# MaxHalford/sorobn

Measured on NVIDIA H100. Metric: exact-inference queries/sec, higher is better.
Workload: dtype f32

## Files before the change

### sorobn_b200/csrc/sbn_join.cu

```cuda
#include "sbn_join.h"

#include <cuda.h>

#include <algorithm>
#include <cstring>

#include "sbn_internal.h"
#include "sbn_kernels.cuh"
#include "sbn_launch.h"
#include "sbn_tma.h"

namespace {

constexpr int kT = 5;
constexpr int kSmemMax = 220 * 1024;

struct SbnJoinParams {
    CUtensorMap tm[SBN_JOIN_MAX_BATCHED];
    SbnStep s;
    int32_t boff[SBN_MAX_IN];
    int32_t map_in[SBN_JOIN_MAX_BATCHED];
    int32_t n_maps;
    int32_t rows;
    int32_t stage_floats;
    uint32_t stage_bytes;
    int32_t n_blocks;
};

__device__ __forceinline__ void tma_3d(float *dst, const CUtensorMap *map, int32_t row, uint64_t *bar) {
    asm volatile("cp.async.bulk.tensor.3d.shared::cluster.global.mbarrier::complete_tx::bytes [%0], [%1, {%3, %4, %4}], [%2];" ::"r"(
                     sbn_smem_u32(dst)),
                 "l"(reinterpret_cast<uint64_t>(map)), "r"(sbn_smem_u32(bar)), "r"(row), "r"(0)
                 : "memory");
}

template <int NU, int NA, int NB>
__global__ void __launch_bounds__(SBN_JOIN_MAX_THREADS, 1) sbn_join_kernel(const __grid_constant__ SbnJoinParams p) {
    constexpr int T = kT, CX = kT, S = SBN_JOIN_STAGES;
    constexpr int N_IN = NU + NA + NB;
    constexpr int TB = NB > 0 ? T : 1;
    constexpr int ROW_WORDS = N_IN + 2;
    const SbnStep &s = p.s;
    extern __shared__ __align__(128) float s_mem[];
    __shared__ __align__(8) uint64_t s_full[S], s_tab;
    sbn_pdl_launch_dependents();

    const int R = p.rows;
    float *const tab = s_mem + S * p.stage_floats;
    const bool staged = s.smem_floats > 0;
    if (threadIdx.x == 0) {
#pragma unroll
        for (int k = 0; k < S; ++k) sbn_mbar_init(&s_full[k], 1);
        sbn_mbar_init(&s_tab, 1);
        sbn_fence_mbar_init();
    }
    __syncthreads();
    if (threadIdx.x == 0 && staged) {
        sbn_mbar_expect_tx(&s_tab, static_cast<uint32_t>(s.smem_floats) * 4u);
#pragma unroll
        for (int i = 0; i < N_IN; ++i)
            if (!s.in[i].batched) sbn_tma_bulk_g2s(tab + s.in[i].smem_off, s.in[i].ptr, static_cast<uint32_t>(s.in[i].stage_floats) * 4u, &s_tab);
    }
    auto issue = [&](int stage, int blk) {
        float *const dst = s_mem + stage * p.stage_floats;
        sbn_mbar_expect_tx(&s_full[stage], p.stage_bytes);
        for (int m = 0; m < p.n_maps; ++m) tma_3d(dst + p.boff[p.map_in[m]], &p.tm[m], blk * R, &s_full[stage]);
    };
    sbn_pdl_wait();
    if (threadIdx.x == 0)
        for (int k = 0; k < S; ++k)
            if (blockIdx.x + k * gridDim.x < p.n_blocks) issue(k, blockIdx.x + k * gridDim.x);

    const int r = threadIdx.x % R, t = threadIdx.x / R;
    const int32_t *const row = s.tile_off + static_cast<int64_t>(t) * ROW_WORDS;
    const int o_base = __ldg(row);
    int base[N_IN];
#pragma unroll
    for (int i = 0; i < N_IN; ++i) base[i] = __ldg(row + 2 + i);
    const int c0 = s.card[0];
    const int cx = s.cx;
    if (staged) sbn_mbar_wait(&s_tab, 0);

    for (int it = 0, blk = blockIdx.x; blk < p.n_blocks; ++it, blk += gridDim.x) {
        const int stage = it % S;
        const int b = blk * R + r;
        const bool live = b < s.n_rows;
        const float *src[N_IN];
        int mul[N_IN];
        const float *const stg = s_mem + stage * p.stage_floats;
#pragma unroll
        for (int i = 0; i < N_IN; ++i) {
            if (s.in[i].batched) {
                src[i] = stg + p.boff[i] + r;
                mul[i] = R;
            } else {
                int e = s.in[i].smem_off;
                for (int k = 0; k < s.in[i].n_ev; ++k) {
                    const int code = live ? min(static_cast<int>(s.ev[static_cast<int64_t>(s.in[i].ev_col[k]) * s.ld_ev + b]), s.in[i].ev_card[k] - 1) : 0;
                    e += code * s.in[i].ev_stride[k];
                }
                src[i] = tab + e;
                mul[i] = 1;
            }
        }
        sbn_mbar_wait(&s_full[stage], static_cast<uint32_t>((it / S) & 1));

        float acc[T][TB];
#pragma unroll
        for (int d0 = 0; d0 < T; ++d0)
#pragma unroll
            for (int d1 = 0; d1 < TB; ++d1) acc[d0][d1] = 0.f;
        for (int xo = 0; xo < cx; xo += CX) {
            int ob[N_IN];
#pragma unroll
            for (int i = 0; i < N_IN; ++i) ob[i] = base[i] + __ldg(s.zoff + i * cx + xo);
#pragma unroll
            for (int x = 0; x < CX; ++x) {
                float a[T], bb[TB];
#pragma unroll
                for (int d = 0; d < T; ++d) {
                    float v = 1.f;
#pragma unroll
                    for (int j = 0; j < NA; ++j) {
                        const int i = NU + j;
                        const float r_ = src[i][(ob[i] + x * s.in[i].sx + d * s.in[i].stride[0]) * mul[i]];
                        v = (j == 0) ? r_ : v * r_;
                    }
#pragma unroll
                    for (int i = 0; i < NU; ++i) v *= src[i][(ob[i] + x * s.in[i].sx) * mul[i]];
                    a[d] = v;
                }
#pragma unroll
                for (int d = 0; d < TB; ++d) {
                    float v = 1.f;
#pragma unroll
                    for (int j = 0; j < NB; ++j) {
                        const int i = NU + NA + j;
                        const float r_ = src[i][(ob[i] + x * s.in[i].sx + d * s.in[i].stride[1]) * mul[i]];
                        v = (j == 0) ? r_ : v * r_;
                    }
                    bb[d] = v;
                }
#pragma unroll
                for (int d0 = 0; d0 < T; ++d0)
#pragma unroll
                    for (int d1 = 0; d1 < TB; ++d1) acc[d0][d1] = fmaf(a[d0], bb[d1], acc[d0][d1]);
            }
        }
        if (live) {
#pragma unroll
            for (int d1 = 0; d1 < TB; ++d1)
#pragma unroll
                for (int d0 = 0; d0 < T; ++d0) __stcs(s.out + static_cast<int64_t>(o_base + d1 * c0 + d0) * s.ld + b, acc[d0][d1]);
        }
        __syncthreads();
        if (threadIdx.x == 0 && blk + S * static_cast<int>(gridDim.x) < p.n_blocks) issue(stage, blk + S * gridDim.x);
    }
}

#define SBN_JOIN_COMBOS(X) \
    X(0, 1, 0) X(0, 1, 1) X(0, 1, 2) X(0, 2, 0) X(0, 2, 1) X(1, 1, 0) X(1, 1, 1) X(1, 2, 0) X(2, 1, 0) X(2, 1, 1)

bool instantiated(int nu, int na, int nb) {
#define SBN_JOIN_HAS(U, A, B) \
    if (nu == U && na == A && nb == B) return true;
    SBN_JOIN_COMBOS(SBN_JOIN_HAS)
#undef SBN_JOIN_HAS
    return false;
}

struct JoinShape {
    int rows = 0;
    int stage_floats = 0;
    uint32_t stage_bytes = 0;
    size_t smem = 0;
    int32_t boff[SBN_MAX_IN] = {};
    int e_lo[SBN_MAX_IN] = {};
};

int split_entries(int64_t n) {
    for (int d = 256; d >= 1; --d)
        if (n % d == 0) return n / d <= 256 ? d : 0;
    return 0;
}

bool shape_of(const sbn_program *P, const StepDesc &st, const SbnStep &q, JoinShape *js) {
    if (P->f64 || !P->use_tiled || !P->use_preload) return false;
    if (st.kind != 1 || st.tile != kT || st.nc != 0 || q.tile_off == nullptr || q.zoff == nullptr || q.cx_inner != kT || q.cx % kT != 0)
        return false;
    if (q.slab_off != nullptr || q.slices != nullptr || q.norm_out != nullptr) return false;
    if (!(st.in.size() <= 3 || (st.nu == 2 && st.na == 1 && st.nb == 1)) || !instantiated(st.nu, st.na, st.nb)) return false;
    const int64_t n_tiles = st.n_tiles;
    const int tb = st.nb > 0 ? kT : 1;
    for (int64_t t = 0; t < n_tiles; ++t)
        if (P->h_tile_words[static_cast<size_t>(st.tile_off_pos + t * (q.n_in + 2) + 1)] != (kT | tb << 8)) return false;
    const int rows = n_tiles * 16 >= 128 ? 16 : 32;
    if (n_tiles * rows < 128 || n_tiles * rows > SBN_JOIN_MAX_THREADS) return false;
    int n_batched = 0;
    int64_t stage = 0;
    for (int i = 0; i < q.n_in; ++i) {
        const InDesc &in = st.in[st.order[i]];
        if (!in.batched) {
            if (q.in[i].smem_off < 0) return false;
            continue;
        }
        if (++n_batched > SBN_JOIN_MAX_BATCHED) return false;
        const int64_t n_e = P->slots[in.id].size;
        js->e_lo[i] = split_entries(n_e);
        if (js->e_lo[i] == 0) return false;
        js->boff[i] = static_cast<int32_t>(stage);
        stage += round_up(n_e * rows, 32);
        js->stage_bytes += static_cast<uint32_t>(n_e * rows * 4);
    }
    if (n_batched != SBN_JOIN_MAX_BATCHED) return false;
    js->rows = rows;
    js->stage_floats = static_cast<int>(stage);
    js->smem = static_cast<size_t>(SBN_JOIN_STAGES * stage + q.smem_floats) * 4;
    if (js->smem > kSmemMax) return false;
    return q.n_rows >= 2LL * P->n_sms * rows;
}

template <int NU, int NA, int NB>
cudaError_t set_attr() {
    return cudaFuncSetAttribute(sbn_join_kernel<NU, NA, NB>, cudaFuncAttributeMaxDynamicSharedMemorySize, kSmemMax);
}

}

int sbn_join_rows(const sbn_program *P, const StepDesc &st, const SbnStep &q) {
    JoinShape js;
    return shape_of(P, st, q, &js) ? js.rows : 0;
}

cudaError_t sbn_join_set_attrs() {
    cudaError_t e = cudaSuccess;
#define SBN_JOIN_ATTR(U, A, B) \
    if (e == cudaSuccess) e = set_attr<U, A, B>();
    SBN_JOIN_COMBOS(SBN_JOIN_ATTR)
#undef SBN_JOIN_ATTR
    return e;
}

cudaError_t sbn_join_launch(sbn_program *P, const StepDesc &st, const SbnStep &q, cudaStream_t stream) {
    JoinShape js;
    if (!shape_of(P, st, q, &js)) return cudaErrorInvalidValue;
    SbnJoinParams p;
    memset(&p, 0, sizeof p);
    p.s = q;
    p.rows = js.rows;
    p.stage_floats = js.stage_floats;
    p.stage_bytes = js.stage_bytes;
    p.n_blocks = static_cast<int32_t>((q.n_rows + js.rows - 1) / js.rows);
    for (int i = 0; i < q.n_in; ++i) {
        p.boff[i] = js.boff[i];
        if (!q.in[i].batched) continue;
        const int64_t n_e = P->slots[st.in[st.order[i]].id].size;
        if (!sbn_tma_encode_rows(&p.tm[p.n_maps], q.in[i].ptr, q.ld, q.n_rows, n_e, js.rows, js.e_lo[i])) return cudaErrorInvalidValue;
        p.map_in[p.n_maps++] = i;
    }
    const dim3 g(static_cast<unsigned>(std::min<int64_t>(p.n_blocks, P->n_sms))), b(static_cast<unsigned>(js.rows * st.n_tiles));
    const int key = st.nu * 100 + st.na * 10 + st.nb;
    switch (key) {
#define SBN_JOIN_CASE(U, A, B)                                                \
    case U * 100 + A * 10 + B:                                                \
        sbn_launch(sbn_join_kernel<U, A, B>, g, b, js.smem, stream, p);       \
        break;
        SBN_JOIN_COMBOS(SBN_JOIN_CASE)
#undef SBN_JOIN_CASE
        default: return cudaErrorInvalidValue;
    }
    return cudaGetLastError();
}
```

Measured before the change: 26.53 million.

## Stage join outputs in shared memory and write them with TMA bulk stores

Output tiles are now written into a shared-memory box and sent to global memory with a TMA tensor store, replacing per-thread streaming stores. The next block's inputs are prefetched into L2 with TMA, and evidence columns are prefetched with prefetch.global.L2. Addressing is also rewritten to precomputed byte offsets with strength-reduced x increments. This uses more shared memory, adds an extra __syncthreads per block, and requires the output entry count to be splittable.

Result: faster. 27.33 million, median of 6 (+3.0%).

```diff
diff --git a/sorobn_b200/csrc/sbn_join.cu b/sorobn_b200/csrc/sbn_join.cu
--- a/sorobn_b200/csrc/sbn_join.cu
+++ b/sorobn_b200/csrc/sbn_join.cu
@@ -17,12 +17,14 @@
 
 struct SbnJoinParams {
     CUtensorMap tm[SBN_JOIN_MAX_BATCHED];
+    CUtensorMap tm_out;
     SbnStep s;
     int32_t boff[SBN_MAX_IN];
     int32_t map_in[SBN_JOIN_MAX_BATCHED];
     int32_t n_maps;
     int32_t rows;
     int32_t stage_floats;
+    int32_t out_floats;
     uint32_t stage_bytes;
     int32_t n_blocks;
 };
@@ -32,6 +34,18 @@
                      sbn_smem_u32(dst)),
                  "l"(reinterpret_cast<uint64_t>(map)), "r"(sbn_smem_u32(bar)), "r"(row), "r"(0)
                  : "memory");
+}
+
+__device__ __forceinline__ void tma_prefetch_3d(const CUtensorMap *map, int32_t row) {
+    asm volatile("cp.async.bulk.prefetch.tensor.3d.L2.global [%0, {%1, %2, %2}];" ::"l"(reinterpret_cast<uint64_t>(map)), "r"(row), "r"(0)
+                 : "memory");
+}
+
+__device__ __forceinline__ void tma_store_3d(const CUtensorMap *map, const float *src, int32_t row) {
+    asm volatile("cp.async.bulk.tensor.3d.global.shared::cta.bulk_group [%0, {%2, %3, %3}], [%1];" ::"l"(reinterpret_cast<uint64_t>(map)),
+                 "r"(sbn_smem_u32(src)), "r"(row), "r"(0)
+                 : "memory");
+    asm volatile("cp.async.bulk.commit_group;" ::: "memory");
 }
 
 template <int NU, int NA, int NB>
@@ -46,7 +60,8 @@
     sbn_pdl_launch_dependents();
 
     const int R = p.rows;
-    float *const tab = s_mem + S * p.stage_floats;
+    float *const obox = s_mem + S * p.stage_floats;
+    float *const tab = obox + p.out_floats;
     const bool staged = s.smem_floats > 0;
     if (threadIdx.x == 0) {
 #pragma unroll
@@ -66,41 +81,60 @@
         sbn_mbar_expect_tx(&s_full[stage], p.stage_bytes);
         for (int m = 0; m < p.n_maps; ++m) tma_3d(dst + p.boff[p.map_in[m]], &p.tm[m], blk * R, &s_full[stage]);
     };
+    auto prefetch = [&](int blk) {
+        for (int m = 0; m < p.n_maps; ++m) tma_prefetch_3d(&p.tm[m], blk * R);
+    };
     sbn_pdl_wait();
-    if (threadIdx.x == 0)
+    if (threadIdx.x == 0) {
         for (int k = 0; k < S; ++k)
             if (blockIdx.x + k * gridDim.x < p.n_blocks) issue(k, blockIdx.x + k * gridDim.x);
+        if (blockIdx.x + S * gridDim.x < p.n_blocks) prefetch(blockIdx.x + S * gridDim.x);
+    }
 
     const int r = threadIdx.x % R, t = threadIdx.x / R;
     const int32_t *const row = s.tile_off + static_cast<int64_t>(t) * ROW_WORDS;
     const int o_base = __ldg(row);
-    int base[N_IN];
-#pragma unroll
-    for (int i = 0; i < N_IN; ++i) base[i] = __ldg(row + 2 + i);
+    const int tab_b = static_cast<int>(tab - s_mem) * 4;
+    int tile_b[N_IN], mb[N_IN], xs_b[N_IN], ds_b[N_IN];
+    const int32_t *zp[N_IN];
+#pragma unroll
+    for (int i = 0; i < N_IN; ++i) {
+        const bool bat = s.in[i].batched != 0;
+        mb[i] = bat ? 4 * R : 4;
+        tile_b[i] = __ldg(row + 2 + i) * mb[i] + (bat ? (p.boff[i] + r) * 4 : tab_b + s.in[i].smem_off * 4);
+        xs_b[i] = s.in[i].sx * mb[i];
+        ds_b[i] = (i < NU ? 0 : i < NU + NA ? s.in[i].stride[0] : s.in[i].stride[1]) * mb[i];
+        zp[i] = s.zoff + i * s.cx;
+    }
     const int c0 = s.card[0];
     const int cx = s.cx;
+    const char *const smc = reinterpret_cast<const char *>(s_mem);
+    auto ld = [&](int off) { return *reinterpret_cast<const float *>(smc + off); };
     if (staged) sbn_mbar_wait(&s_tab, 0);
 
     for (int it = 0, blk = blockIdx.x; blk < p.n_blocks; ++it, blk += gridDim.x) {
         const int stage = it % S;
         const int b = blk * R + r;
         const bool live = b < s.n_rows;
-        const float *src[N_IN];
-        int mul[N_IN];
-        const float *const stg = s_mem + stage * p.stage_floats;
+        if (t == 0 && b + static_cast<int>(gridDim.x) * R < s.n_rows) {
+#pragma unroll
+            for (int i = 0; i < N_IN; ++i)
+                if (!s.in[i].batched)
+                    for (int k = 0; k < s.in[i].n_ev; ++k)
+                        asm volatile("prefetch.global.L2 [%0];" ::"l"(s.ev + static_cast<int64_t>(s.in[i].ev_col[k]) * s.ld_ev + b + gridDim.x * R));
+        }
+        int blk_off[N_IN];
 #pragma unroll
         for (int i = 0; i < N_IN; ++i) {
             if (s.in[i].batched) {
-                src[i] = stg + p.boff[i] + r;
-                mul[i] = R;
+                blk_off[i] = tile_b[i] + stage * p.stage_floats * 4;
             } else {
-                int e = s.in[i].smem_off;
+                int e = 0;
                 for (int k = 0; k < s.in[i].n_ev; ++k) {
                     const int code = live ? min(static_cast<int>(s.ev[static_cast<int64_t>(s.in[i].ev_col[k]) * s.ld_ev + b]), s.in[i].ev_card[k] - 1) : 0;
                     e += code * s.in[i].ev_stride[k];
                 }
-                src[i] = tab + e;
-                mul[i] = 1;
+                blk_off[i] = tile_b[i] + e * 4;
             }
         }
         sbn_mbar_wait(&s_full[stage], static_cast<uint32_t>((it / S) & 1));
@@ -113,7 +147,7 @@
         for (int xo = 0; xo < cx; xo += CX) {
             int ob[N_IN];
 #pragma unroll
-            for (int i = 0; i < N_IN; ++i) ob[i] = base[i] + __ldg(s.zoff + i * cx + xo);
+            for (int i = 0; i < N_IN; ++i) ob[i] = blk_off[i] + __ldg(zp[i] + xo) * mb[i];
 #pragma unroll
             for (int x = 0; x < CX; ++x) {
                 float a[T], bb[TB];
@@ -123,11 +157,11 @@
 #pragma unroll
                     for (int j = 0; j < NA; ++j) {
                         const int i = NU + j;
-                        const float r_ = src[i][(ob[i] + x * s.in[i].sx + d * s.in[i].stride[0]) * mul[i]];
+                        const float r_ = ld(ob[i] + d * ds_b[i]);
                         v = (j == 0) ? r_ : v * r_;
                     }
 #pragma unroll
-                    for (int i = 0; i < NU; ++i) v *= src[i][(ob[i] + x * s.in[i].sx) * mul[i]];
+                    for (int i = 0; i < NU; ++i) v *= ld(ob[i]);
                     a[d] = v;
                 }
 #pragma unroll
@@ -136,7 +170,7 @@
 #pragma unroll
                     for (int j = 0; j < NB; ++j) {
                         const int i = NU + NA + j;
-                        const float r_ = src[i][(ob[i] + x * s.in[i].sx + d * s.in[i].stride[1]) * mul[i]];
+                        const float r_ = ld(ob[i] + d * ds_b[i]);
                         v = (j == 0) ? r_ : v * r_;
                     }
                     bb[d] = v;
@@ -145,17 +179,26 @@
                 for (int d0 = 0; d0 < T; ++d0)
 #pragma unroll
                     for (int d1 = 0; d1 < TB; ++d1) acc[d0][d1] = fmaf(a[d0], bb[d1], acc[d0][d1]);
+#pragma unroll
+                for (int i = 0; i < N_IN; ++i) ob[i] += xs_b[i];
             }
         }
-        if (live) {
-#pragma unroll
-            for (int d1 = 0; d1 < TB; ++d1)
-#pragma unroll
-                for (int d0 = 0; d0 < T; ++d0) __stcs(s.out + static_cast<int64_t>(o_base + d1 * c0 + d0) * s.ld + b, acc[d0][d1]);
-        }
+        if (threadIdx.x == 0) asm volatile("cp.async.bulk.wait_group.read 0;" ::: "memory");
         __syncthreads();
-        if (threadIdx.x == 0 && blk + S * static_cast<int>(gridDim.x) < p.n_blocks) issue(stage, blk + S * gridDim.x);
-    }
+        if (threadIdx.x == 0) {
+            const int nxt = blk + S * static_cast<int>(gridDim.x);
+            if (nxt < p.n_blocks) issue(stage, nxt);
+            if (nxt + static_cast<int>(gridDim.x) < p.n_blocks) prefetch(nxt + gridDim.x);
+        }
+#pragma unroll
+        for (int d1 = 0; d1 < TB; ++d1)
+#pragma unroll
+            for (int d0 = 0; d0 < T; ++d0) obox[(o_base + d1 * c0 + d0) * R + r] = acc[d0][d1];
+        asm volatile("fence.proxy.async.shared::cta;" ::: "memory");
+        __syncthreads();
+        if (threadIdx.x == 0) tma_store_3d(&p.tm_out, obox, blk * R);
+    }
+    if (threadIdx.x == 0) asm volatile("cp.async.bulk.wait_group 0;" ::: "memory");
 }
 
 #define SBN_JOIN_COMBOS(X) \
@@ -176,6 +219,8 @@
     size_t smem = 0;
     int32_t boff[SBN_MAX_IN] = {};
     int e_lo[SBN_MAX_IN] = {};
+    int out_lo = 0;
+    int out_floats = 0;
 };
 
 int split_entries(int64_t n) {
@@ -215,7 +260,10 @@
     if (n_batched != SBN_JOIN_MAX_BATCHED) return false;
     js->rows = rows;
     js->stage_floats = static_cast<int>(stage);
-    js->smem = static_cast<size_t>(SBN_JOIN_STAGES * stage + q.smem_floats) * 4;
+    js->out_lo = split_entries(q.n_out);
+    if (js->out_lo == 0) return false;
+    js->out_floats = static_cast<int>(round_up(static_cast<int64_t>(q.n_out) * rows, 32));
+    js->smem = static_cast<size_t>(SBN_JOIN_STAGES * stage + js->out_floats + q.smem_floats) * 4;
     if (js->smem > kSmemMax) return false;
     return q.n_rows >= 2LL * P->n_sms * rows;
 }
@@ -258,6 +306,8 @@
         if (!sbn_tma_encode_rows(&p.tm[p.n_maps], q.in[i].ptr, q.ld, q.n_rows, n_e, js.rows, js.e_lo[i])) return cudaErrorInvalidValue;
         p.map_in[p.n_maps++] = i;
     }
+    if (!sbn_tma_encode_rows(&p.tm_out, q.out, q.ld, q.n_rows, q.n_out, js.rows, js.out_lo)) return cudaErrorInvalidValue;
+    p.out_floats = js.out_floats;
     const dim3 g(static_cast<unsigned>(std::min<int64_t>(p.n_blocks, P->n_sms))), b(static_cast<unsigned>(js.rows * st.n_tiles));
     const int key = st.nu * 100 + st.na * 10 + st.nb;
     switch (key) {
```
